# ShawnHuang497/MedPLIB

Hardware: AMD Instinct MI355X
Metric: train samples/sec (img+64tok) (higher is better)
Workload: dtype bf16

## Files before the change

### include/medplib_hip.h

```cpp
#ifndef MEDPLIB_HIP_H
#define MEDPLIB_HIP_H
#include <stddef.h>
#include <stdint.h>

#ifdef __cplusplus
extern "C" {
#endif

typedef struct ihipStream_t* hipStream_t;

#define MP_OK 0
#define MP_ERR_SHAPE (-1)
#define MP_ERR_DTYPE (-2)
#define MP_ERR_WORKSPACE (-3)
#define MP_ERR_LAUNCH (-4)
#define MP_ERR_ARG (-5)
#define MP_BF16 0
#define MP_F32 1
#define MP_ACT_NONE 0
#define MP_ACT_RELU 1
#define MP_ACT_GELU 2
#define MP_ACT_QUICK_GELU 3
#define MP_ACT_SILU 4
#define MP_ACT_SWIGLU_PAIR 5
// ... 48 lines not shown
#define MP_POS_ERR_CACHE 2
int mp_gemv_rmsnorm_rope_append_bounded_bf16(const void* x, int64_t ldx, const float* norm_w, float eps, const void* W_qkv, int64_t ldw,
                                             void* qkv, int64_t ldy, const float* cos_t, const float* sin_t, void* cache_k, void* cache_v,
                                             const int* pos_dev, int M, int heads, int head_dim, int K, int64_t cache_batch_stride,
                                             int64_t cache_seq_stride, int table_rows, int cache_rows, int* err, hipStream_t stream);

int mp_gemm_set_workspace(void* ws, int64_t ws_bytes, int* tickets, int n_tickets);
int mp_gemm_set_stream_workspace(hipStream_t stream, void* ws, int64_t ws_bytes, int* tickets, int n_tickets);

int mp_attention_fwd_bf16(const void* Q, int64_t q_sb, int64_t q_ss, const void* K, int64_t k_sb, int64_t k_ss,
                          const void* V, int64_t v_sb, int64_t v_ss, void* O, int64_t o_sb, int64_t o_ss,
                          const uint8_t* key_valid, const float* rel_h, const float* rel_w, int kh, int kw, int B, int H,
                          int Sq, int Sk, int D, int causal, float scale, int variant, const int* sk_dev, hipStream_t stream);

int mp_rmsnorm_bf16(const void* x, int64_t ldx, const float* w, void* y, int64_t ldy, int64_t rows, int dim, float eps,
                    hipStream_t stream);
int mp_layernorm_bf16(const void* x, int64_t ldx, const float* w, const float* b, void* y, int64_t ldy, int64_t rows,
                      int dim, float eps, hipStream_t stream);
int mp_rope_qk_bf16(void* qkv, int64_t ld, const float* cos_t, const float* sin_t, int64_t tokens, int seq, int heads,
                    int head_dim, int pos_offset, hipStream_t stream);
int mp_rope_qk_bounded_bf16(void* qkv, int64_t ld, const float* cos_t, const float* sin_t, int64_t tokens, int seq, int heads,
                            int head_dim, int pos_offset, int table_rows, hipStream_t stream);
int mp_decode_rope_append_bf16(void* qkv, int64_t ld, const float* cos_t, const float* sin_t, void* cache_k, void* cache_v,
                               const int* pos_dev, int B, int heads, int head_dim, int64_t cache_batch_stride, int64_t cache_seq_stride,
                               hipStream_t stream);
int mp_decode_rope_append_bounded_bf16(void* qkv, int64_t ld, const float* cos_t, const float* sin_t, void* cache_k, void* cache_v,
                                       const int* pos_dev, int B, int heads, int head_dim, int64_t cache_batch_stride,
                                       int64_t cache_seq_stride, int table_rows, int cache_rows, int* err, hipStream_t stream);
int mp_advance_ints(int* p, int n, int delta, hipStream_t stream);
int mp_argmax_rows_f32(const float* x, int64_t ld, int64_t rows, int cols, int64_t* out, hipStream_t stream);
int mp_sample_rows_f32(const float* logits, int64_t ld, int64_t rows, int cols, float inv_temperature, const float* u, int64_t* out,
// ... 109 lines not shown
int mp_decode_norm_gate_route(const void* x, int64_t ldx, const float* ln_w, float eps, const float* wg, void* h, int64_t ldh,
                              const float* rts_uniform, int tokens, int dim, int n_experts, int capacity, float* gates, int* expert,
                              int* slot, float* weight, int* kept_counts, long long* exp_counts, float* l_aux, hipStream_t stream);
int mp_decode_norm_gate_route_top2(const void* x, int64_t ldx, const float* ln_w, float eps, const float* wg, void* h, int64_t ldh,
                                   const float* noise, int tokens, int dim, int n_experts, int capacity, int* expert, int* slot,
                                   float* weight, int* kept_counts, long long* exp_counts, float* l_aux, hipStream_t stream);
int mp_moe_residual_mix_bf16(const void* x, const void* moe, const void* mlp, const void* coef, int64_t ldcoef, void* out,
                             int64_t tokens, int dim, hipStream_t stream);
int mp_moe_route_top2(const float* gates, const float* logits, const float* noise, int tokens, int n_experts, int capacity,
                      int* expert, int* slot, float* weight, int* kept_counts, long long* exp_counts, float* l_aux,
                      hipStream_t stream);
int mp_gate_noise_f32(float* out, int64_t n, uint64_t seed, uint64_t offset, int gumbel, hipStream_t stream);
int mp_gate_noise_dev_f32(float* out, int64_t n, uint64_t seed, const int* pass_dev, uint64_t stride, int gumbel, hipStream_t stream);
int mp_rmsnorm_gate_bf16(const void* x, int64_t ldx, const float* ln_w, float eps, void* h, int64_t ldh, const float* wg, float* logits,
                         float* gates, int64_t tokens, int dim, int n_experts, hipStream_t stream);
int mp_rmsnorm_gate_rstd_bf16(const void* x, int64_t ldx, const float* ln_w, float eps, const float* wg, float* logits, float* gates,
                              float* rstd, int64_t tokens, int dim, int n_experts, hipStream_t stream);
int mp_gemm_qkv_rope_scaled_bf16(const void* A, int64_t lda, const void* Wi, int64_t ldw, void* C, int64_t ldc, const float* cos_t,
                                 const float* sin_t, const float* row_scale, int M, int N, int K, int seq, int pos_offset, int head_dim,
                                 hipStream_t stream);
int mp_gemm_qkv_rope_scaled_bounded_bf16(const void* A, int64_t lda, const void* Wi, int64_t ldw, void* C, int64_t ldc, const float* cos_t,
                                         const float* sin_t, const float* row_scale, int M, int N, int K, int seq, int pos_offset,
                                         int head_dim, int table_rows, hipStream_t stream);
int mp_gemm_bf16_nt_batched_rows_scaled(const void* A, int64_t lda, const int* a_rows, const float* a_row_scale, const void* W, int64_t ldw,
                                        int64_t strideW, void* C, int64_t ldc, int64_t strideC, int rows_stride, int batch, int M, int N,
                                        int K, const int* m_dev, hipStream_t stream);
int mp_gemm_fold_ok(int M, int N, int K);
int mp_moe_dispatch_bf16(const void* x, int64_t ldx, const int* expert, const int* slot, void* buf, int64_t ldbuf, int64_t tokens, int dim,
                         int capacity, int top_k, hipStream_t stream);
int mp_moe_combine_bf16(const void* y, const int* expert, const int* slot, const float* weight, const void* residual, void* out,
// ... 114 lines not shown
```

### medplib_amd/csrc/ce_moe.hip

```cpp
#include "common.h"
#include <algorithm>

namespace {

constexpr int MAXE = 8;

__global__ __launch_bounds__(256) void ce_rows_kernel(const float* __restrict__ logits, int64_t ld, const int64_t* __restrict__ labels,
                                                      int V, float* __restrict__ row_loss) {
  __shared__ float red[16];
  const int64_t r = blockIdx.x;
  const float* x = logits + r * ld;
  float m = -INFINITY;
  for (int i = threadIdx.x; i < V; i += 256) m = fmaxf(m, x[i]);
  m = block_max(m, red);
  float s = 0.f;
  for (int i = threadIdx.x; i < V; i += 256) s += expf(x[i] - m);
  s = block_sum(s, red);
  if (threadIdx.x == 0) row_loss[r] = logf(s) + m - x[labels[r]];
}

__global__ __launch_bounds__(256) void mean_plus_kernel(const float* __restrict__ x, int64_t n, float scale, const float* __restrict__ add,
                                                        int n_add, float add_scale, float* __restrict__ out) {
  __shared__ float red[16];
  float s = 0.f;
// ... 39 lines not shown
        for (int j = 0; j < 8; ++j) acc[e] = fmaf((float)v[j], w[j], acc[e]);
      }
    }
  }
  moe_gate_finish(acc, E, lane, logits_out, gates_out);
}

__global__ __launch_bounds__(256) void moe_gate_kernel(const bf16_t* __restrict__ x, int64_t ldx, const float* __restrict__ wg,
                                                       float* __restrict__ logits, float* __restrict__ gates, int64_t T, int d, int E) {
  const int lane = threadIdx.x & 63;
  const int64_t tok = (int64_t)blockIdx.x * 4 + (threadIdx.x >> 6);
  if (tok >= T) return;
  moe_gate_token(x + tok * ldx, wg, d, E, lane, logits + tok * E, gates + tok * E);
}

template <int NCH, bool LDSW>
__global__ __launch_bounds__(512) void rmsnorm_gate_kernel(const bf16_t* __restrict__ x, int64_t ldx, const float* __restrict__ w, float eps,
                                                           bf16_t* __restrict__ h, int64_t ldh, const float* __restrict__ wg, int E,
                                                           float* __restrict__ logits, float* __restrict__ gates, int64_t T, float* __restrict__ rstd = nullptr) {
  extern __shared__ __attribute__((aligned(16))) float wsh[];
  constexpr int dim = NCH * 512;
  const int lane = threadIdx.x & 63;
  const int nwv = blockDim.x >> 6, step4 = blockDim.x * 4;
  if constexpr (LDSW) {
    for (int i = threadIdx.x * 4; i < dim; i += step4) *reinterpret_cast<f32x4*>(wsh + i) = *reinterpret_cast<const f32x4*>(w + i);
    for (int i = threadIdx.x * 4; i < E * dim; i += step4) *reinterpret_cast<f32x4*>(wsh + dim + i) = *reinterpret_cast<const f32x4*>(wg + i);
    __syncthreads();
  }
  const float* wn = LDSW ? wsh : w;
  const float* wgs = LDSW ? wsh + dim : wg;
  for (int64_t tok = (int64_t)blockIdx.x * nwv + (threadIdx.x >> 6); tok < T; tok += (int64_t)gridDim.x * nwv) {
    const bf16_t* xr = x + tok * ldx;
    bf16x8 v[NCH];
    float part[4] = {0.f, 0.f, 0.f, 0.f};
#pragma unroll
    for (int k = 0; k < NCH; ++k) {
      v[k] = *reinterpret_cast<const bf16x8*>(xr + (k * 64 + lane) * 8);
#pragma unroll
      for (int j = 0; j < 8; ++j) { const float f = (float)v[k][j]; part[k & 3] += f * f; }
    }
    float ss = 0.f;
#pragma unroll
    for (int wv = 0; wv < 4; ++wv) ss += wave_sum(part[wv]);
    const float rs = rsqrtf(ss / (float)dim + eps);
    if (rstd && lane == 0) rstd[tok] = rs;
    if (!h && E == 0) continue;
    float acc[MAXE];
#pragma unroll
    for (int e = 0; e < MAXE; ++e) acc[e] = 0.f;
    bf16_t* hr = h + tok * ldh;
#pragma unroll
    for (int k = 0; k < NCH; ++k) {
// ... 20 lines not shown
    float mx = -INFINITY;
#pragma unroll
    for (int e = 0; e < MAXE; ++e)
      if (e < E) { acc[e] = wave_sum(acc[e]); mx = fmaxf(mx, acc[e]); }
    if (lane == 0) {
      float sum = 0.f, pr[MAXE];
#pragma unroll
      for (int e = 0; e < MAXE; ++e)
        if (e < E) { pr[e] = expf(acc[e] - mx); sum += pr[e]; }
#pragma unroll
      for (int e = 0; e < MAXE; ++e)
        if (e < E) {
          if (logits) logits[tok * E + e] = acc[e];
          gates[tok * E + e] = pr[e] / sum;
        }
    }
  }
}

template <bool FAST>
__global__ __launch_bounds__(1024) void moe_route_top1_kernel(const float* __restrict__ gates, const float* __restrict__ rts, int T,
                                                              int E, int capacity, int* __restrict__ expert, int* __restrict__ slot,
                                                              float* __restrict__ weight, int* __restrict__ kept_counts,
                                                              long long* __restrict__ exp_counts, float* __restrict__ l_aux,
                                                              int* __restrict__ slot_token) {
  __shared__ float red[16];
  __shared__ int cnt_sh[MAXE];
  __shared__ int scan[16][MAXE];
  const int tid = threadIdx.x;
  if (tid < MAXE) cnt_sh[tid] = 0;
  __syncthreads();
  float me[MAXE];
  int cnt[MAXE];
#pragma unroll
  for (int e = 0; e < MAXE; ++e) { me[e] = 0.f; cnt[e] = 0; }
  const int chunk = (T + 1023) / 1024;
  const int s0 = min(T, tid * chunk), s1 = min(T, s0 + chunk);
  int ex[FAST ? 16 : 1];
  if constexpr (FAST) {
    float bvv[16];
// ... 40 lines not shown
    }
  }
  float aux = 0.f;
  for (int e = 0; e < E; ++e) {
    float m = 0.f; int c = 0;
#pragma unroll
    for (int k = 0; k < MAXE; ++k) if (k == e) { m = me[k]; c = cnt[k]; }
    const float msum = block_sum(m, red);
    int cw = c;
#pragma unroll
    for (int off = 1; off < 64; off <<= 1) cw += __shfl_xor(cw, off, 64);
    if ((tid & 63) == 0 && cw) atomicAdd(&cnt_sh[e], cw);
    __syncthreads();
    aux += (msum / (float)T) * ((float)cnt_sh[e] / (float)T);
  }
  if (tid == 0) {
    l_aux[0] = aux * (float)E;
    for (int e = 0; e < E; ++e) exp_counts[e] = cnt_sh[e];
  }
  __syncthreads();
  const int lane = tid & 63, wv = tid >> 6;
  bool over = false;
  for (int e = 0; e < E; ++e) over |= cnt_sh[e] > capacity;
  const bool via_memory = !FAST || (rts && over);
  if (via_memory) {
    for (int s = tid; s < T; s += 1024) slot[s] = 1;
    __syncthreads();
  }
  if (rts && over) {
    __shared__ unsigned hist[256];
    __shared__ unsigned bin_suf[256], bin_tot[4];
// ... 158 lines not shown
    }
    if (kp) {
      int v = 0;
#pragma unroll
      for (int k = 0; k < MAXE; ++k) if (k == e) { v = base[k]; base[k] += 1; }
      slot[s] = (v < capacity) ? v : -1;
      if (slot_token && v < capacity) slot_token[(int64_t)e * capacity + v] = s;
    } else {
      slot[s] = -1;
    }
  }
  if (tid == 1023)
    for (int e = 0; e < E; ++e) kept_counts[e] = min(base[e], capacity);
}

__device__ __forceinline__ void moe_route_top1_small_body(const float* __restrict__ gates, const float* __restrict__ rts, int T,
                                                               int E, int capacity, int* __restrict__ expert, int* __restrict__ slot,
                                                                  float* __restrict__ weight, int* __restrict__ kept_counts,
                                                                  long long* __restrict__ exp_counts, float* __restrict__ l_aux,
                                                                  int* __restrict__ slot_token, int s) {
  const bool live = s < T;
  int best = 0;
  float bv = live ? gates[(int64_t)s * E] : 0.f;
  float aux = 0.f;
  for (int e = 1; e < E; ++e) {
    const float g = live ? gates[(int64_t)s * E + e] : 0.f;
    if (g > bv) { bv = g; best = e; }
  }
  for (int e = 0; e < E; ++e) {
    const float me = wave_sum(live ? gates[(int64_t)s * E + e] : 0.f) / (float)T;
// ... 425 lines not shown
extern "C" int mp_mean_plus_f32(const float* x, int64_t n, float scale, const float* add, int n_add, float add_scale, float* out,
                                hipStream_t stream) {
  hipLaunchKernelGGL(mean_plus_kernel, dim3(1), dim3(256), 0, stream, x, n, scale, add, n_add, add_scale, out);
  return mp_check_launch("mp_mean_plus_f32");
}

extern "C" int mp_moe_gate_bf16(const void* x, int64_t ldx, const float* wg, float* logits, float* gates, int64_t tokens, int dim,
                                int n_experts, hipStream_t stream) {
  MP_REQUIRE(n_experts >= 1 && n_experts <= MAXE && dim % 8 == 0 && ldx % 8 == 0, MP_ERR_SHAPE, "mp_moe_gate_bf16: bad shape (E<=8)");
  if (tokens == 0) return MP_OK;
  hipLaunchKernelGGL(moe_gate_kernel, dim3((unsigned)mp_cdiv(tokens, 4)), dim3(256), 0, stream, (const bf16_t*)x, ldx, wg, logits,
                     gates, tokens, dim, n_experts);
  return mp_check_launch("mp_moe_gate_bf16");
}

static int rmsnorm_gate_launch(const void* x, int64_t ldx, const float* ln_w, float eps, void* h, int64_t ldh, const float* wg,
                                    float* logits, float* gates, int64_t tokens, int dim, int n_experts, float* rstd, hipStream_t stream) {
  MP_REQUIRE(n_experts >= 0 && n_experts <= MAXE && ldx % 8 == 0 && ldh % 8 == 0, MP_ERR_SHAPE, "mp_rmsnorm_gate_bf16: bad shape (E <= %d)", MAXE);
  MP_REQUIRE(dim == 2048 || dim == 4096 || dim == 8192, MP_ERR_SHAPE, "mp_rmsnorm_gate_bf16: dim %d (2048, 4096 or 8192)", dim);
  MP_REQUIRE(n_experts == 0 || (wg != nullptr && gates != nullptr), MP_ERR_ARG, "mp_rmsnorm_gate_bf16: gate outputs missing");
  if (tokens == 0) return MP_OK;
  const size_t lds = (size_t)(1 + n_experts) * dim * sizeof(float);
  const bool stage = lds <= 65536;
  static int rg_waves = -1;
  if (rg_waves < 0) { const char* e = getenv("MP_RG_WAVES"); rg_waves = (e && atoi(e) == 8) ? 8 : 4; }
  const int nwv = (stage && tokens >= 2048) ? rg_waves : 4;
  const dim3 grid((unsigned)std::min<int64_t>(mp_cdiv(tokens, nwv), stage ? (nwv == 8 ? 768 : 512) : (1 << 30))), blk(64 * nwv);
#define MP_RG(N)                                                                                                                                   \
  do {                                                                                                                                             \
    if (stage) hipLaunchKernelGGL((rmsnorm_gate_kernel<N, true>), grid, blk, lds, stream, (const bf16_t*)x, ldx, ln_w, eps, (bf16_t*)h, ldh, wg,   \
                                  n_experts, logits, gates, tokens, rstd);                                                                               \
    else hipLaunchKernelGGL((rmsnorm_gate_kernel<N, false>), grid, blk, 0, stream, (const bf16_t*)x, ldx, ln_w, eps, (bf16_t*)h, ldh, wg,          \
                            n_experts, logits, gates, tokens, rstd);                                                                                     \
  } while (0)
  if (dim == 2048) MP_RG(4); else if (dim == 4096) MP_RG(8); else MP_RG(16);
#undef MP_RG
  return mp_check_launch("mp_rmsnorm_gate_bf16");
}

extern "C" int mp_rmsnorm_gate_bf16(const void* x, int64_t ldx, const float* ln_w, float eps, void* h, int64_t ldh, const float* wg, float* logits,
                                    float* gates, int64_t tokens, int dim, int n_experts, hipStream_t stream) {
  MP_REQUIRE(h != nullptr, MP_ERR_ARG, "mp_rmsnorm_gate_bf16: h is null (mp_rmsnorm_gate_rstd_bf16 is the form without the normalised rows)");
  return rmsnorm_gate_launch(x, ldx, ln_w, eps, h, ldh, wg, logits, gates, tokens, dim, n_experts, nullptr, stream);
}

extern "C" int mp_rmsnorm_gate_rstd_bf16(const void* x, int64_t ldx, const float* ln_w, float eps, const float* wg, float* logits, float* gates,
                                         float* rstd, int64_t tokens, int dim, int n_experts, hipStream_t stream) {
  MP_REQUIRE(rstd != nullptr && ln_w != nullptr, MP_ERR_ARG, "mp_rmsnorm_gate_rstd_bf16: rstd and ln_w required");
  return rmsnorm_gate_launch(x, ldx, ln_w, eps, nullptr, 8, wg, logits, gates, tokens, dim, n_experts, rstd, stream);
}

extern "C" int mp_moe_route_top1(const float* gates, const float* rts_uniform, int tokens, int n_experts, int capacity, int* expert,
                                 int* slot, float* weight, int* kept_counts, long long* exp_counts, float* l_aux, int* slot_token,
                                 hipStream_t stream) {
  MP_REQUIRE(n_experts >= 1 && n_experts <= MAXE && tokens > 0 && capacity >= 0, MP_ERR_SHAPE, "mp_moe_route_top1: bad shape");
  if (tokens <= 64) {
    hipLaunchKernelGGL(moe_route_top1_small_kernel, dim3(1), dim3(64), 0, stream, gates, rts_uniform, tokens, n_experts, capacity, expert,
                       slot, weight, kept_counts, exp_counts, l_aux, slot_token);
    return mp_check_launch("mp_moe_route_top1(small)");
  }
  if (tokens <= 16 * 1024)
    hipLaunchKernelGGL(moe_route_top1_kernel<true>, dim3(1), dim3(1024), 0, stream, gates, rts_uniform, tokens, n_experts, capacity, expert,
                       slot, weight, kept_counts, exp_counts, l_aux, slot_token);
  else
    hipLaunchKernelGGL(moe_route_top1_kernel<false>, dim3(1), dim3(1024), 0, stream, gates, rts_uniform, tokens, n_experts, capacity, expert,
                       slot, weight, kept_counts, exp_counts, l_aux, slot_token);
  return mp_check_launch("mp_moe_route_top1");
}

extern "C" int mp_decode_norm_gate_route(const void* x, int64_t ldx, const float* ln_w, float eps, const float* wg, void* h, int64_t ldh,
                                        const float* rts_uniform, int tokens, int dim, int n_experts, int capacity, float* gates,
                                        int* expert, int* slot, float* weight, int* kept_counts, long long* exp_counts, float* l_aux,
                                        hipStream_t stream) {
  MP_REQUIRE(tokens >= 1 && tokens <= 8 && n_experts >= 1 && n_experts <= MAXE && dim % 8 == 0 && dim <= 8192 && ldx % 8 == 0 &&
                 ldh % 8 == 0 && capacity >= 0,
             MP_ERR_SHAPE, "mp_decode_norm_gate_route: tokens <= 8, experts <= %d, dim %% 8 == 0 and <= 8192", MAXE);
  hipLaunchKernelGGL(decode_norm_gate_route_kernel, dim3(1), dim3(256), 0, stream, (const bf16_t*)x, ldx, ln_w, eps, wg, (bf16_t*)h, ldh,
                     rts_uniform, tokens, dim, n_experts, capacity, gates, expert, slot, weight, kept_counts, exp_counts, l_aux);
  return mp_check_launch("mp_decode_norm_gate_route");
}

extern "C" int mp_decode_norm_gate_route_top2(const void* x, int64_t ldx, const float* ln_w, float eps, const float* wg, void* h, int64_t ldh,
// ... 78 lines not shown
```

### medplib_amd/csrc/norm_elementwise.hip

```cpp
#include "common.h"

namespace {

constexpr int ROW_THREADS = 256;
constexpr int MAXC = 4;

__global__ __launch_bounds__(ROW_THREADS) void rmsnorm_bf16_kernel(const bf16_t* __restrict__ x, const float* __restrict__ w,
                                                                   bf16_t* __restrict__ y, int dim, float eps,
                                                                   int64_t ldx, int64_t ldy) {
  __shared__ float red[16];
  const int64_t row = blockIdx.x;
  const bf16_t* xr = x + row * ldx;
  bf16_t* yr = y + row * ldy;
  bf16x8 v[MAXC];
  float ss = 0.f;
#pragma unroll
  for (int c = 0; c < MAXC; ++c) {
    const int i = (c * ROW_THREADS + threadIdx.x) * 8;
    if (i < dim) {
      v[c] = *reinterpret_cast<const bf16x8*>(xr + i);
#pragma unroll
      for (int j = 0; j < 8; ++j) { const float f = (float)v[c][j]; ss += f * f; }
    }
  }
  ss = block_sum(ss, red);
  const float rs = rsqrtf(ss / (float)dim + eps);
// ... 301 lines not shown
}

}

extern "C" int mp_argmax_rows_f32(const float* x, int64_t ld, int64_t rows, int cols, int64_t* out, hipStream_t stream) {
  MP_REQUIRE(cols > 0, MP_ERR_SHAPE, "mp_argmax_rows_f32: bad shape");
  if (rows == 0) return MP_OK;
  if (cols <= 32768)
    hipLaunchKernelGGL(argmax_rows_wide_kernel, dim3((unsigned)rows), dim3(1024), 0, stream, x, ld, cols, out);
  else
    hipLaunchKernelGGL(argmax_rows_kernel, dim3((unsigned)rows), dim3(256), 0, stream, x, ld, cols, out);
  return mp_check_launch("mp_argmax_rows_f32");
}

extern "C" int mp_rmsnorm_bf16(const void* x, int64_t ldx, const float* w, void* y, int64_t ldy, int64_t rows, int dim,
                               float eps, hipStream_t stream) {
  MP_REQUIRE(dim % 8 == 0 && dim <= ROW_THREADS * 8 * MAXC && ldx % 8 == 0 && ldy % 8 == 0, MP_ERR_SHAPE,
             "mp_rmsnorm_bf16: dim=%d unsupported", dim);
  if (rows == 0) return MP_OK;
  hipLaunchKernelGGL(rmsnorm_bf16_kernel, dim3((unsigned)rows), dim3(ROW_THREADS), 0, stream, (const bf16_t*)x, w,
                     (bf16_t*)y, dim, eps, ldx, ldy);
  return mp_check_launch("mp_rmsnorm_bf16");
}

extern "C" int mp_layernorm_bf16(const void* x, int64_t ldx, const float* w, const float* b, void* y, int64_t ldy,
                                 int64_t rows, int dim, float eps, hipStream_t stream) {
  MP_REQUIRE(dim % 8 == 0 && dim <= ROW_THREADS * 8 * MAXC && ldx % 8 == 0 && ldy % 8 == 0, MP_ERR_SHAPE,
             "mp_layernorm_bf16: dim=%d unsupported", dim);
  if (rows == 0) return MP_OK;
  if (dim <= 2048) {
    hipLaunchKernelGGL(layernorm_bf16_wave_kernel, dim3((unsigned)mp_cdiv(rows, 4)), dim3(256), 0, stream, (const bf16_t*)x, w, b,
                       (bf16_t*)y, rows, dim, eps, ldx, ldy);
    return mp_check_launch("mp_layernorm_bf16");
  }
  hipLaunchKernelGGL(layernorm_bf16_kernel, dim3((unsigned)rows), dim3(ROW_THREADS), 0, stream, (const bf16_t*)x, w, b,
                     (bf16_t*)y, dim, eps, ldx, ldy);
// ... 101 lines not shown
```

### medplib_amd/model/llama.py

```python
import math

import torch

from .. import ops


def _rope_tables(seq, head_dim, theta, device, start=0):
    inv = 1.0 / (theta ** (torch.arange(0, head_dim, 2, dtype=torch.float32) / head_dim))
    freqs = torch.outer(torch.arange(start, seq, dtype=torch.float32), inv)
    return freqs.cos().contiguous().to(device), freqs.sin().contiguous().to(device)


ROPE_GROW_ROWS = 1024


def rope_rows_for(n, rows):
    return rows if n <= rows else -(-n // ROPE_GROW_ROWS) * ROPE_GROW_ROWS


class LlamaStack:
    def __init__(self, cfg, device, init_std=0.02, seed=0):
        self.cfg, self.device = cfg, device
        d, ff, L, V = cfg.hidden_size, cfg.intermediate_size, cfg.num_hidden_layers, cfg.vocab_size
        E = cfg.num_experts
# ... 134 lines not shown
        if self.rts_uniform_provider is not None:
            return self.rts_uniform_provider(i, T, E)
        if not self.cfg.moe_gate_sampling:
            return None
        L = len(self.layers)
        pass_dev = self._pass_dev
        key = (self.gate_pass, T, E, bool(gumbel), pass_dev is not None)
        if getattr(self, "_draws_key", None) != key:
            if pass_dev is not None:
                self._draws_all = ops.gate_noise_dev(L * T * E, self.cfg.moe_gate_seed, pass_dev, L * T * E, gumbel, self.device)
            else:
                self._draws_all = ops.gate_noise(L * T * E, self.cfg.moe_gate_seed, self.gate_pass * L * T * E, gumbel, self.device)
            self._draws_key = key
        return self._draws_all[i * T * E:(i + 1) * T * E]

    def _mlp(self, i, lw, h, x, gate=None, needed=None, rstd=None):
        cfg = self.cfg
        T = x.shape[0]
        if i not in self.moe_layers:
            if T <= 8:
                return ops.gemv(ops.gemv(h, lw["gu"], act=ops.ACT_SWIGLU_PAIR), lw["down"], residual=x), None, None
            act = ops.gemm(h, lw["gu"], act=ops.ACT_SWIGLU_PAIR)
            return ops.gemm(act, lw["down"], residual=x), None, None
        E, ff, d = cfg.num_experts, cfg.intermediate_size, cfg.hidden_size
        cap = self.capacity(T)
        k = cfg.top_k_experts
        logits, gates = gate if gate is not None else ops.moe_gate(h, lw["wg"])
        if k == 1 and self.ep is None and T <= 8 and not cfg.use_residual:
            draws = None if cap >= T else self._gate_draws(i, T, E, gumbel=False)
            expert, slot, weight, kept, counts, l_aux = ops.moe_route_top1(gates, cap, draws)
            act = ops.gemv(h, lw["gu"], act=ops.ACT_SWIGLU_PAIR, w_index=expert)
            out = ops.gemv(act, lw["down"], residual=x, w_index=expert, row_scale=weight, row_keep=slot)
            return out, l_aux, (expert, slot, counts)
        if k == 2 and self.ep is None and T <= 8 and not cfg.use_residual:
            expert, slot, weight, kept, counts, l_aux = ops.moe_route_top2(gates, logits, cap, self._gate_draws(i, T, E, gumbel=True))
            act = ops.gemv_top2_gate_up(h, lw["gu"], expert, slot)
            return ops.gemv_top2_down(act, lw["down"], expert, slot, weight, x), l_aux, (expert, slot, counts)
        if k == 1 and self.ep is None and self.fuse_moe_gather_scatter and not cfg.use_residual:
            expert, slot, weight, kept, counts, l_aux, slot_token = ops.moe_route_top1(
                gates, cap, self._gate_draws(i, T, E, gumbel=False), want_slot_token=True)
            act = torch.empty((E, cap, ff), dtype=torch.bfloat16, device=x.device)
            if needed is not None:
                self.pruned_rows = int(getattr(self, "needed_rows")[0].numel())
                slot_token, kept = ops.moe_filter_slots(slot_token, kept, needed)
            if ops.GEMM_TIMER is not None:
                ops.GEMM_TIMER.batched_tag = i
            ev = getattr(self, "layer_events", None)
            if ev is not None and i < len(ev):
                ev[i].record()
            if rstd is not None:
                ops.gemm_batched_rows(x, lw["gu_f"], act, kept, a_rows=slot_token, act=ops.ACT_SWIGLU_PAIR, rows_stride=cap, a_row_scale=rstd)
            else:
                ops.gemm_batched_rows(h, lw["gu"], act, kept, a_rows=slot_token, act=ops.ACT_SWIGLU_PAIR, rows_stride=cap)
            ops.gemm_batched_rows(act, lw["down"], x, kept, c_rows=slot_token, c_scale=weight, residual=x, rows_stride=cap)
# ... 98 lines not shown
            else:
                qkv = lin(h, lw["qkv"])
                ops.rope_qk_(qkv, self.cos, self.sin, S, H, D, pos_offset=pos0)
            q5 = qkv.unflatten(0, (B, S)).unflatten(2, (3, H, D))
            if kv_cache is not None:
                kv_cache["k"][i][:, pos0:pos0 + S].copy_(q5[:, :, 1])
                kv_cache["v"][i][:, pos0:pos0 + S].copy_(q5[:, :, 2])
            if kv_cache is not None and pos0 > 0:
                assert S == 1 and key_valid is None, "cached decode is single-token, un-padded (the reference evaluates with batch 1)"
                attn = ops.attention(q5[:, :, 0], kv_cache["k"][i][:, :pos0 + 1], kv_cache["v"][i][:, :pos0 + 1], causal=False)
            else:
                attn = ops.attention(q5[:, :, 0], q5[:, :, 1], q5[:, :, 2], causal=True, key_valid=key_valid)
            x = lin(attn.view(B * S, d), lw["o"], residual=x)
            x_gate_in = x.clone() if (collect_routing and i in self.moe_layers) else None
            if i in self.moe_layers and d in ops.RMSNORM_GATE_DIMS and B * S > 8:
                h, lg, gt = ops.rmsnorm_gate(x, lw["ln2"], cfg.rms_norm_eps, lw["wg"])
                x, l_aux, r = self._mlp(i, lw, h, x, gate=(lg, gt), needed=needed_mask if i == len(self.layers) - 1 else None)
            else:
                h = ops.rmsnorm(x, lw["ln2"], cfg.rms_norm_eps)
                x, l_aux, r = self._mlp(i, lw, h, x, needed=needed_mask if (i in self.moe_layers and i == len(self.layers) - 1) else None)
            if l_aux is not None:
                aux.append(l_aux)
                if collect_routing:
                    routing.append(r)
                    gate_inputs.append(x_gate_in)
        if kv_cache is not None:
            kv_cache["len"] = pos0 + S
        out = ops.rmsnorm(x, self.norm_w, cfg.rms_norm_eps)
        if collect_routing:
            self.last_gate_inputs = gate_inputs
        return out.view(B, S, d), aux, (routing if collect_routing else None)

    def decode_step(self, emb, kv_cache, counters, pass_dev=None):
        self._pass_dev = pass_dev
        try:
            return self._decode_step(emb, kv_cache, counters)
        finally:
            self._pass_dev = None

    def _decode_step(self, emb, kv_cache, counters):
        cfg = self.cfg
        B, _, d = emb.shape
        H, D = cfg.num_attention_heads, cfg.head_dim
# ... 53 lines not shown
```

### medplib_amd/ops.py

```python
import torch

from ._lib import lib

BF16, F32 = 0, 1
ACT_NONE, ACT_RELU, ACT_GELU, ACT_QUICK_GELU, ACT_SILU, ACT_SWIGLU_PAIR = 0, 1, 2, 3, 4, 5
SACT_NONE, SACT_RELU, SACT_GELU, SACT_SIGMOID = 0, 1, 2, 3


def _stream():
    return torch.cuda.current_stream().cuda_stream


def _p(t):
    return None if t is None else t.data_ptr()


def _chk(t, dtype, name):
    if not t.is_cuda:
        raise ValueError(f"{name}: expected a GPU tensor (medplib_amd has no CPU path)")
    if t.dtype != dtype:
        raise TypeError(f"{name}: expected {dtype}, got {t.dtype}")


def _dt(dtype):
# ... 622 lines not shown
    return cos_t.shape[0], cache_k.shape[1], err


def decode_rope_append(qkv, cos_t, sin_t, cache_k, cache_v, pos_dev, heads, head_dim, err=None):
    _chk(qkv, torch.bfloat16, "decode_rope_append.qkv"); _chk(pos_dev, torch.int32, "decode_rope_append.pos")
    assert qkv.dim() == 2 and qkv.stride(1) == 1 and cache_k.stride(3) == 1 and cache_k.stride(2) == head_dim
    table_rows, cache_rows, err = _decode_bounds(cos_t, sin_t, cache_k, cache_v, err)
    lib().call("mp_decode_rope_append_bounded_bf16", _p(qkv), qkv.stride(0), _p(cos_t), _p(sin_t), _p(cache_k), _p(cache_v), _p(pos_dev),
               qkv.shape[0], heads, head_dim, cache_k.stride(0), cache_k.stride(1), table_rows, cache_rows, _p(err), _stream())


def advance_ints(t, delta=1):
    lib().call("mp_advance_ints", _p(t), t.numel(), int(delta), _stream())


def rmsnorm(x, w, eps, out=None):
    _chk(x, torch.bfloat16, "rmsnorm.x"); _chk(w, torch.float32, "rmsnorm.w")
    x2 = x.reshape(-1, x.shape[-1]); assert x2.stride(1) == 1
    if out is None:
        out = torch.empty_like(x2)
    lib().call("mp_rmsnorm_bf16", _p(x2), x2.stride(0), _p(w), _p(out), out.stride(0), x2.shape[0], x2.shape[1], float(eps),
               _stream())
    return out.view(x.shape)


def layernorm(x, w, b, eps, out=None):
    _chk(x, torch.bfloat16, "layernorm.x"); _chk(w, torch.float32, "layernorm.w")
    x2 = x.reshape(-1, x.shape[-1]); assert x2.stride(1) == 1
    if out is None:
        out = torch.empty_like(x2)
    lib().call("mp_layernorm_bf16", _p(x2), x2.stride(0), _p(w), _p(b), _p(out), out.stride(0), x2.shape[0], x2.shape[1],
               float(eps), _stream())
    return out.view(x.shape)


def rope_qk_(qkv, cos_t, sin_t, seq, heads, head_dim, pos_offset=0):
    _chk(qkv, torch.bfloat16, "rope.qkv"); _chk(cos_t, torch.float32, "rope.cos"); _chk(sin_t, torch.float32, "rope.sin")
# ... 635 lines not shown
def moe_route_top1(gates, capacity, rts_uniform=None, want_slot_token=False):
    T, E = gates.shape
    dev = gates.device
    slot_token = torch.empty((E, int(capacity)), dtype=torch.int32, device=dev) if want_slot_token else None
    expert = torch.empty(T, dtype=torch.int32, device=dev); slot = torch.empty(T, dtype=torch.int32, device=dev)
    weight = torch.empty(T, dtype=torch.float32, device=dev)
    kept = torch.empty(E, dtype=torch.int32, device=dev); counts = torch.empty(E, dtype=torch.int64, device=dev)
    l_aux = torch.empty(1, dtype=torch.float32, device=dev)
    lib().call("mp_moe_route_top1", _p(gates), _p(rts_uniform), T, E, int(capacity), _p(expert), _p(slot), _p(weight), _p(kept),
               _p(counts), _p(l_aux), _p(slot_token), _stream())
    if want_slot_token:
        return expert, slot, weight, kept, counts, l_aux, slot_token
    return expert, slot, weight, kept, counts, l_aux


def decode_norm_gate_route(x, ln_w, eps, wg, capacity, rts_uniform=None):
    _chk(x, torch.bfloat16, "decode_norm_gate_route.x"); _chk(ln_w, torch.float32, "decode_norm_gate_route.ln_w")
    _chk(wg, torch.float32, "decode_norm_gate_route.wg")
    T, d = x.shape
    E = wg.shape[0]
    dev = x.device
    h = torch.empty((T, d), dtype=torch.bfloat16, device=dev)
    expert = torch.empty(T, dtype=torch.int32, device=dev); slot = torch.empty(T, dtype=torch.int32, device=dev)
    weight = torch.empty(T, dtype=torch.float32, device=dev)
    kept = torch.empty(E, dtype=torch.int32, device=dev); counts = torch.empty(E, dtype=torch.int64, device=dev)
    l_aux = torch.empty(1, dtype=torch.float32, device=dev)
    lib().call("mp_decode_norm_gate_route", _p(x), x.stride(0), _p(ln_w), float(eps), _p(wg), _p(h), h.stride(0), _p(rts_uniform), T, d, E,
               int(capacity), None, _p(expert), _p(slot), _p(weight), _p(kept), _p(counts), _p(l_aux), _stream())
    return h, expert, slot, weight, kept, counts, l_aux

# ... 202 lines not shown
```

Measured before the change: 138.0.

## Fuse top-1 MoE routing into rmsnorm-gate kernel and normalize only needed rows

Extends the rmsnorm+gate kernel with a ROUTE variant that computes argmax expert, weight and per-workgroup count/gate-sum partials in the same pass. A new multi-block ranges kernel then derives global counts, aux loss and capacity slots with ballot-based ranking, falling back to the serial router when random token selection is needed. Each workgroup now owns a contiguous row range and prefetches its first row before staging weights. The final rmsnorm takes an optional row index list so only the needed rows are normalized. This removes a separate single-block routing pass and some final-norm work, at the cost of a workspace buffer and more complex partitioning logic.

New measurement: 137.9 (median of 2 runs). Within noise of the previous version (-0.0%).

```diff
diff --git a/include/medplib_hip.h b/include/medplib_hip.h
--- a/include/medplib_hip.h
+++ b/include/medplib_hip.h
@@ -86,7 +86,7 @@
                           int Sq, int Sk, int D, int causal, float scale, int variant, const int* sk_dev, hipStream_t stream);
 
 int mp_rmsnorm_bf16(const void* x, int64_t ldx, const float* w, void* y, int64_t ldy, int64_t rows, int dim, float eps,
-                    hipStream_t stream);
+                    const int64_t* row_idx, hipStream_t stream);
 int mp_layernorm_bf16(const void* x, int64_t ldx, const float* w, const float* b, void* y, int64_t ldy, int64_t rows,
                       int dim, float eps, hipStream_t stream);
 int mp_rope_qk_bf16(void* qkv, int64_t ld, const float* cos_t, const float* sin_t, int64_t tokens, int seq, int heads,
@@ -226,6 +226,12 @@
 int mp_gate_noise_dev_f32(float* out, int64_t n, uint64_t seed, const int* pass_dev, uint64_t stride, int gumbel, hipStream_t stream);
 int mp_rmsnorm_gate_bf16(const void* x, int64_t ldx, const float* ln_w, float eps, void* h, int64_t ldh, const float* wg, float* logits,
                          float* gates, int64_t tokens, int dim, int n_experts, hipStream_t stream);
+#define MP_ROUTE_MAX_WGS 1024
+#define MP_ROUTE_WS_BYTES (MP_ROUTE_MAX_WGS * 8 * 12)
+int mp_rmsnorm_gate_route_top1_bf16(const void* x, int64_t ldx, const float* ln_w, float eps, void* h, int64_t ldh, const float* wg,
+                                    float* logits, float* gates, const float* rts_uniform, int tokens, int dim, int n_experts,
+                                    int capacity, int* expert, int* slot, float* weight, int* kept_counts, long long* exp_counts,
+                                    float* l_aux, int* slot_token, void* workspace, int64_t workspace_bytes, hipStream_t stream);
 int mp_rmsnorm_gate_rstd_bf16(const void* x, int64_t ldx, const float* ln_w, float eps, const float* wg, float* logits, float* gates,
                               float* rstd, int64_t tokens, int dim, int n_experts, hipStream_t stream);
 int mp_gemm_qkv_rope_scaled_bf16(const void* A, int64_t lda, const void* Wi, int64_t ldw, void* C, int64_t ldc, const float* cos_t,
diff --git a/medplib_amd/csrc/ce_moe.hip b/medplib_amd/csrc/ce_moe.hip
--- a/medplib_amd/csrc/ce_moe.hip
+++ b/medplib_amd/csrc/ce_moe.hip
@@ -4,6 +4,8 @@
 namespace {
 
 constexpr int MAXE = 8;
+constexpr int MP_ROUTE_MAX_WGS = 1024;
+constexpr int64_t MP_ROUTE_WS_BYTES = (int64_t)MP_ROUTE_MAX_WGS * MAXE * 12;
 
 __global__ __launch_bounds__(256) void ce_rows_kernel(const float* __restrict__ logits, int64_t ld, const int64_t* __restrict__ labels,
                                                       int V, float* __restrict__ row_loss) {
@@ -77,14 +79,31 @@
   moe_gate_token(x + tok * ldx, wg, d, E, lane, logits + tok * E, gates + tok * E);
 }
 
-template <int NCH, bool LDSW>
+struct RoutePartials {
+  int* expert;
+  float* weight;
+  int* cnt;
+  double* gsum;
+};
+
+template <int NCH, bool LDSW, bool ROUTE>
 __global__ __launch_bounds__(512) void rmsnorm_gate_kernel(const bf16_t* __restrict__ x, int64_t ldx, const float* __restrict__ w, float eps,
                                                            bf16_t* __restrict__ h, int64_t ldh, const float* __restrict__ wg, int E,
-                                                           float* __restrict__ logits, float* __restrict__ gates, int64_t T, float* __restrict__ rstd = nullptr) {
+                                                           float* __restrict__ logits, float* __restrict__ gates, int64_t T, int rows_wg,
+                                                           float* __restrict__ rstd, RoutePartials rp) {
   extern __shared__ __attribute__((aligned(16))) float wsh[];
+  __shared__ int cnt_wv[8][MAXE];
+  __shared__ double gsum_wv[8][MAXE];
   constexpr int dim = NCH * 512;
   const int lane = threadIdx.x & 63;
   const int nwv = blockDim.x >> 6, step4 = blockDim.x * 4;
+  const int64_t row_end = min(T, ((int64_t)blockIdx.x + 1) * rows_wg);
+  int64_t tok = (int64_t)blockIdx.x * rows_wg + (threadIdx.x >> 6);
+  bf16x8 v[NCH];
+  if (tok < row_end) {
+#pragma unroll
+    for (int k = 0; k < NCH; ++k) v[k] = *reinterpret_cast<const bf16x8*>(x + tok * ldx + (k * 64 + lane) * 8);
+  }
   if constexpr (LDSW) {
     for (int i = threadIdx.x * 4; i < dim; i += step4) *reinterpret_cast<f32x4*>(wsh + i) = *reinterpret_cast<const f32x4*>(w + i);
     for (int i = threadIdx.x * 4; i < E * dim; i += step4) *reinterpret_cast<f32x4*>(wsh + dim + i) = *reinterpret_cast<const f32x4*>(wg + i);
@@ -92,13 +111,16 @@
   }
   const float* wn = LDSW ? wsh : w;
   const float* wgs = LDSW ? wsh + dim : wg;
-  for (int64_t tok = (int64_t)blockIdx.x * nwv + (threadIdx.x >> 6); tok < T; tok += (int64_t)gridDim.x * nwv) {
+  int rcnt[MAXE];
+  double rsum[MAXE];
+#pragma unroll
+  for (int e = 0; e < MAXE; ++e) { rcnt[e] = 0; rsum[e] = 0.0; }
+  for (bool first = true; tok < row_end; tok += nwv, first = false) {
     const bf16_t* xr = x + tok * ldx;
-    bf16x8 v[NCH];
     float part[4] = {0.f, 0.f, 0.f, 0.f};
 #pragma unroll
     for (int k = 0; k < NCH; ++k) {
-      v[k] = *reinterpret_cast<const bf16x8*>(xr + (k * 64 + lane) * 8);
+      if (!first) v[k] = *reinterpret_cast<const bf16x8*>(xr + (k * 64 + lane) * 8);
 #pragma unroll
       for (int j = 0; j < 8; ++j) { const float f = (float)v[k][j]; part[k & 3] += f * f; }
     }
@@ -149,16 +171,46 @@
           if (logits) logits[tok * E + e] = acc[e];
           gates[tok * E + e] = pr[e] / sum;
         }
+      if constexpr (ROUTE) {
+        int best = 0;
+        float bv = pr[0] / sum;
+#pragma unroll
+        for (int e = 0; e < MAXE; ++e)
+          if (e < E) {
+            const float g = pr[e] / sum;
+            if (e > 0 && g > bv) { bv = g; best = e; }
+            rsum[e] += (double)g;
+          }
+        rp.expert[tok] = best;
+        rp.weight[tok] = bv;
+#pragma unroll
+        for (int e = 0; e < MAXE; ++e) rcnt[e] += (e == best);
+      }
+    }
+  }
+  if constexpr (ROUTE) {
+    const int wv = threadIdx.x >> 6;
+    if (lane == 0) {
+#pragma unroll
+      for (int e = 0; e < MAXE; ++e) { cnt_wv[wv][e] = rcnt[e]; gsum_wv[wv][e] = rsum[e]; }
+    }
+    __syncthreads();
+    if ((int)threadIdx.x < E) {
+      int c = 0;
+      double g = 0.0;
+      for (int k = 0; k < nwv; ++k) { c += cnt_wv[k][threadIdx.x]; g += gsum_wv[k][threadIdx.x]; }
+      rp.cnt[(int64_t)blockIdx.x * E + threadIdx.x] = c;
+      rp.gsum[(int64_t)blockIdx.x * E + threadIdx.x] = g;
     }
   }
 }
 
 template <bool FAST>
-__global__ __launch_bounds__(1024) void moe_route_top1_kernel(const float* __restrict__ gates, const float* __restrict__ rts, int T,
-                                                              int E, int capacity, int* __restrict__ expert, int* __restrict__ slot,
-                                                              float* __restrict__ weight, int* __restrict__ kept_counts,
-                                                              long long* __restrict__ exp_counts, float* __restrict__ l_aux,
-                                                              int* __restrict__ slot_token) {
+__device__ __forceinline__ void moe_route_top1_body(const float* __restrict__ gates, const float* __restrict__ rts, int T,
+                                                    int E, int capacity, int* __restrict__ expert, int* __restrict__ slot,
+                                                    float* __restrict__ weight, int* __restrict__ kept_counts,
+                                                    long long* __restrict__ exp_counts, float* __restrict__ l_aux,
+                                                    int* __restrict__ slot_token) {
   __shared__ float red[16];
   __shared__ int cnt_sh[MAXE];
   __shared__ int scan[16][MAXE];
@@ -229,7 +281,7 @@
     __syncthreads();
     aux += (msum / (float)T) * ((float)cnt_sh[e] / (float)T);
   }
-  if (tid == 0) {
+  if (tid == 0 && l_aux) {
     l_aux[0] = aux * (float)E;
     for (int e = 0; e < E; ++e) exp_counts[e] = cnt_sh[e];
   }
@@ -418,6 +470,93 @@
     for (int e = 0; e < E; ++e) kept_counts[e] = min(base[e], capacity);
 }
 
+template <bool FAST>
+__global__ __launch_bounds__(1024) void moe_route_top1_kernel(const float* __restrict__ gates, const float* __restrict__ rts, int T,
+                                                              int E, int capacity, int* __restrict__ expert, int* __restrict__ slot,
+                                                              float* __restrict__ weight, int* __restrict__ kept_counts,
+                                                              long long* __restrict__ exp_counts, float* __restrict__ l_aux,
+                                                              int* __restrict__ slot_token) {
+  moe_route_top1_body<FAST>(gates, rts, T, E, capacity, expert, slot, weight, kept_counts, exp_counts, l_aux, slot_token);
+}
+
+__global__ __launch_bounds__(1024) void moe_route_ranges_kernel(const float* __restrict__ gates, const float* __restrict__ rts, int T, int E,
+                                                                int capacity, const int* __restrict__ pcnt, const double* __restrict__ pgsum,
+                                                                int n_part, int rows_wg, int wgs_per, int* __restrict__ expert,
+                                                                int* __restrict__ slot, float* __restrict__ weight,
+                                                                int* __restrict__ kept_counts, long long* __restrict__ exp_counts,
+                                                                float* __restrict__ l_aux, int* __restrict__ slot_token) {
+  __shared__ int tot_sh[MAXE], base_sh[MAXE];
+  __shared__ int wtot[16][MAXE];
+  __shared__ double dred[16];
+  const int tid = threadIdx.x, lane = tid & 63, wv = tid >> 6;
+  const int part0 = blockIdx.x * wgs_per;
+  if (tid < MAXE) { tot_sh[tid] = 0; base_sh[tid] = 0; }
+  __syncthreads();
+  for (int e = 0; e < E; ++e) {
+    int tot = 0, base = 0;
+    for (int g = tid; g < n_part; g += 1024) {
+      const int c = pcnt[(int64_t)g * E + e];
+      tot += c;
+      if (g < part0) base += c;
+    }
+#pragma unroll
+    for (int off = 1; off < 64; off <<= 1) { tot += __shfl_xor(tot, off, 64); base += __shfl_xor(base, off, 64); }
+    if (lane == 0) {
+      if (tot) atomicAdd(&tot_sh[e], tot);
+      if (base) atomicAdd(&base_sh[e], base);
+    }
+  }
+  __syncthreads();
+  bool over = false;
+  for (int e = 0; e < E; ++e) over |= tot_sh[e] > capacity;
+  const bool select = rts != nullptr && over;
+  if (blockIdx.x == 0) {
+    float aux = 0.f;
+    for (int e = 0; e < E; ++e) {
+      double m = 0.0;
+      for (int g = tid; g < n_part; g += 1024) m += pgsum[(int64_t)g * E + e];
+#pragma unroll
+      for (int off = 1; off < 64; off <<= 1) m += __shfl_xor(m, off, 64);
+      if (lane == 0) dred[wv] = m;
+      __syncthreads();
+      double ms = 0.0;
+      for (int k = 0; k < 16; ++k) ms += dred[k];
+      __syncthreads();
+      aux += ((float)ms / (float)T) * ((float)tot_sh[e] / (float)T);
+    }
+    if (tid == 0) {
+      l_aux[0] = aux * (float)E;
+      for (int e = 0; e < E; ++e) {
+        exp_counts[e] = tot_sh[e];
+        if (!select) kept_counts[e] = min(tot_sh[e], capacity);
+      }
+    }
+  }
+  if (select) {
+    if (blockIdx.x != 0) return;
+    if (T <= 16 * 1024) moe_route_top1_body<true>(gates, rts, T, E, capacity, expert, slot, weight, kept_counts, nullptr, nullptr, slot_token);
+    else moe_route_top1_body<false>(gates, rts, T, E, capacity, expert, slot, weight, kept_counts, nullptr, nullptr, slot_token);
+    return;
+  }
+  const int64_t s0 = (int64_t)part0 * rows_wg;
+  const int64_t s = s0 + tid;
+  const bool live = tid < wgs_per * rows_wg && s < T;
+  const int ex = live ? expert[s] : -1;
+  int rank = 0;
+  for (int e = 0; e < E; ++e) {
+    const unsigned long long m = __ballot(ex == e);
+    if (ex == e) rank = __popcll(m & ((1ull << lane) - 1ull));
+    if (lane == 0) wtot[wv][e] = __popcll(m);
+  }
+  __syncthreads();
+  if (live) {
+    rank += base_sh[ex];
+    for (int k = 0; k < wv; ++k) rank += wtot[k][ex];
+    slot[s] = rank < capacity ? rank : -1;
+    if (slot_token && rank < capacity) slot_token[(int64_t)ex * capacity + rank] = (int)s;
+  }
+}
+
 __device__ __forceinline__ void moe_route_top1_small_body(const float* __restrict__ gates, const float* __restrict__ rts, int T,
                                                                int E, int capacity, int* __restrict__ expert, int* __restrict__ slot,
                                                                   float* __restrict__ weight, int* __restrict__ kept_counts,
@@ -873,40 +1012,56 @@
   return mp_check_launch("mp_moe_gate_bf16");
 }
 
+struct RgShape { bool stage; int nwv, rows_wg; unsigned grid; size_t lds; };
+static RgShape rmsnorm_gate_shape(int64_t tokens, int dim, int n_experts, int64_t max_wgs) {
+  RgShape sh;
+  sh.lds = (size_t)(1 + n_experts) * dim * sizeof(float);
+  sh.stage = sh.lds <= 65536;
+  static int rg_waves = -1;
+  if (rg_waves < 0) { const char* e = getenv("MP_RG_WAVES"); rg_waves = (e && atoi(e) == 8) ? 8 : 4; }
+  sh.nwv = (sh.stage && tokens >= 2048) ? rg_waves : 4;
+  const int64_t wgs = std::min<int64_t>(mp_cdiv(tokens, sh.nwv), sh.stage ? (sh.nwv == 8 ? 768 : 512) : max_wgs);
+  sh.rows_wg = (int)mp_cdiv(tokens, wgs);
+  sh.grid = (unsigned)mp_cdiv(tokens, sh.rows_wg);
+  if (!sh.stage) sh.lds = 0;
+  return sh;
+}
+
 static int rmsnorm_gate_launch(const void* x, int64_t ldx, const float* ln_w, float eps, void* h, int64_t ldh, const float* wg,
-                                    float* logits, float* gates, int64_t tokens, int dim, int n_experts, float* rstd, hipStream_t stream) {
+                                    float* logits, float* gates, int64_t tokens, int dim, int n_experts, float* rstd, const RgShape& sh,
+                                    const RoutePartials* rp, hipStream_t stream) {
   MP_REQUIRE(n_experts >= 0 && n_experts <= MAXE && ldx % 8 == 0 && ldh % 8 == 0, MP_ERR_SHAPE, "mp_rmsnorm_gate_bf16: bad shape (E <= %d)", MAXE);
   MP_REQUIRE(dim == 2048 || dim == 4096 || dim == 8192, MP_ERR_SHAPE, "mp_rmsnorm_gate_bf16: dim %d (2048, 4096 or 8192)", dim);
   MP_REQUIRE(n_experts == 0 || (wg != nullptr && gates != nullptr), MP_ERR_ARG, "mp_rmsnorm_gate_bf16: gate outputs missing");
   if (tokens == 0) return MP_OK;
-  const size_t lds = (size_t)(1 + n_experts) * dim * sizeof(float);
-  const bool stage = lds <= 65536;
-  static int rg_waves = -1;
-  if (rg_waves < 0) { const char* e = getenv("MP_RG_WAVES"); rg_waves = (e && atoi(e) == 8) ? 8 : 4; }
-  const int nwv = (stage && tokens >= 2048) ? rg_waves : 4;
-  const dim3 grid((unsigned)std::min<int64_t>(mp_cdiv(tokens, nwv), stage ? (nwv == 8 ? 768 : 512) : (1 << 30))), blk(64 * nwv);
+  const dim3 grid(sh.grid), blk(64 * sh.nwv);
+  const RoutePartials none = {nullptr, nullptr, nullptr, nullptr};
+#define MP_RG_K(N, S, R)                                                                                                                           \
+  hipLaunchKernelGGL((rmsnorm_gate_kernel<N, S, R>), grid, blk, sh.lds, stream, (const bf16_t*)x, ldx, ln_w, eps, (bf16_t*)h, ldh, wg, n_experts,   \
+                     logits, gates, tokens, sh.rows_wg, rstd, rp ? *rp : none)
 #define MP_RG(N)                                                                                                                                   \
   do {                                                                                                                                             \
-    if (stage) hipLaunchKernelGGL((rmsnorm_gate_kernel<N, true>), grid, blk, lds, stream, (const bf16_t*)x, ldx, ln_w, eps, (bf16_t*)h, ldh, wg,   \
-                                  n_experts, logits, gates, tokens, rstd);                                                                               \
-    else hipLaunchKernelGGL((rmsnorm_gate_kernel<N, false>), grid, blk, 0, stream, (const bf16_t*)x, ldx, ln_w, eps, (bf16_t*)h, ldh, wg,          \
-                            n_experts, logits, gates, tokens, rstd);                                                                                     \
+    if (rp) { if (sh.stage) MP_RG_K(N, true, true); else MP_RG_K(N, false, true); }                                                                \
+    else { if (sh.stage) MP_RG_K(N, true, false); else MP_RG_K(N, false, false); }                                                                 \
   } while (0)
   if (dim == 2048) MP_RG(4); else if (dim == 4096) MP_RG(8); else MP_RG(16);
 #undef MP_RG
+#undef MP_RG_K
   return mp_check_launch("mp_rmsnorm_gate_bf16");
 }
 
 extern "C" int mp_rmsnorm_gate_bf16(const void* x, int64_t ldx, const float* ln_w, float eps, void* h, int64_t ldh, const float* wg, float* logits,
                                     float* gates, int64_t tokens, int dim, int n_experts, hipStream_t stream) {
   MP_REQUIRE(h != nullptr, MP_ERR_ARG, "mp_rmsnorm_gate_bf16: h is null (mp_rmsnorm_gate_rstd_bf16 is the form without the normalised rows)");
-  return rmsnorm_gate_launch(x, ldx, ln_w, eps, h, ldh, wg, logits, gates, tokens, dim, n_experts, nullptr, stream);
+  return rmsnorm_gate_launch(x, ldx, ln_w, eps, h, ldh, wg, logits, gates, tokens, dim, n_experts, nullptr,
+                             rmsnorm_gate_shape(tokens, dim, n_experts, (int64_t)1 << 30), nullptr, stream);
 }
 
 extern "C" int mp_rmsnorm_gate_rstd_bf16(const void* x, int64_t ldx, const float* ln_w, float eps, const float* wg, float* logits, float* gates,
                                          float* rstd, int64_t tokens, int dim, int n_experts, hipStream_t stream) {
   MP_REQUIRE(rstd != nullptr && ln_w != nullptr, MP_ERR_ARG, "mp_rmsnorm_gate_rstd_bf16: rstd and ln_w required");
-  return rmsnorm_gate_launch(x, ldx, ln_w, eps, nullptr, 8, wg, logits, gates, tokens, dim, n_experts, rstd, stream);
+  return rmsnorm_gate_launch(x, ldx, ln_w, eps, nullptr, 8, wg, logits, gates, tokens, dim, n_experts, rstd,
+                             rmsnorm_gate_shape(tokens, dim, n_experts, (int64_t)1 << 30), nullptr, stream);
 }
 
 extern "C" int mp_moe_route_top1(const float* gates, const float* rts_uniform, int tokens, int n_experts, int capacity, int* expert,
@@ -925,6 +1080,28 @@
     hipLaunchKernelGGL(moe_route_top1_kernel<false>, dim3(1), dim3(1024), 0, stream, gates, rts_uniform, tokens, n_experts, capacity, expert,
                        slot, weight, kept_counts, exp_counts, l_aux, slot_token);
   return mp_check_launch("mp_moe_route_top1");
+}
+
+extern "C" int mp_rmsnorm_gate_route_top1_bf16(const void* x, int64_t ldx, const float* ln_w, float eps, void* h, int64_t ldh, const float* wg,
+                                               float* logits, float* gates, const float* rts_uniform, int tokens, int dim, int n_experts,
+                                               int capacity, int* expert, int* slot, float* weight, int* kept_counts, long long* exp_counts,
+                                               float* l_aux, int* slot_token, void* workspace, int64_t workspace_bytes, hipStream_t stream) {
+  MP_REQUIRE(h != nullptr && n_experts >= 1 && n_experts <= MAXE && tokens > 0 && capacity >= 0, MP_ERR_SHAPE, "mp_rmsnorm_gate_route_top1_bf16: bad shape");
+  MP_REQUIRE(workspace != nullptr && workspace_bytes >= MP_ROUTE_WS_BYTES && (uintptr_t)workspace % 8 == 0, MP_ERR_WORKSPACE,
+             "mp_rmsnorm_gate_route_top1_bf16: workspace of MP_ROUTE_WS_BYTES, 8-byte aligned");
+  const RgShape sh = rmsnorm_gate_shape(tokens, dim, n_experts, MP_ROUTE_MAX_WGS);
+  MP_REQUIRE(sh.rows_wg <= 1024 && sh.grid <= MP_ROUTE_MAX_WGS, MP_ERR_SHAPE, "mp_rmsnorm_gate_route_top1_bf16: too many tokens (%d)", tokens);
+  RoutePartials rp;
+  rp.expert = expert; rp.weight = weight;
+  rp.gsum = (double*)workspace;
+  rp.cnt = (int*)((char*)workspace + (size_t)MP_ROUTE_MAX_WGS * MAXE * sizeof(double));
+  const int rc = rmsnorm_gate_launch(x, ldx, ln_w, eps, h, ldh, wg, logits, gates, tokens, dim, n_experts, nullptr, sh, &rp, stream);
+  if (rc != MP_OK) return rc;
+  const int wgs_per = 1024 / sh.rows_wg;
+  hipLaunchKernelGGL(moe_route_ranges_kernel, dim3((unsigned)mp_cdiv(sh.grid, wgs_per)), dim3(1024), 0, stream, gates, rts_uniform, tokens,
+                     n_experts, capacity, rp.cnt, rp.gsum, (int)sh.grid, sh.rows_wg, wgs_per, expert, slot, weight, kept_counts, exp_counts,
+                     l_aux, slot_token);
+  return mp_check_launch("mp_rmsnorm_gate_route_top1_bf16");
 }
 
 extern "C" int mp_decode_norm_gate_route(const void* x, int64_t ldx, const float* ln_w, float eps, const float* wg, void* h, int64_t ldh,
diff --git a/medplib_amd/csrc/norm_elementwise.hip b/medplib_amd/csrc/norm_elementwise.hip
--- a/medplib_amd/csrc/norm_elementwise.hip
+++ b/medplib_amd/csrc/norm_elementwise.hip
@@ -7,9 +7,9 @@
 
 __global__ __launch_bounds__(ROW_THREADS) void rmsnorm_bf16_kernel(const bf16_t* __restrict__ x, const float* __restrict__ w,
                                                                    bf16_t* __restrict__ y, int dim, float eps,
-                                                                   int64_t ldx, int64_t ldy) {
+                                                                   int64_t ldx, int64_t ldy, const int64_t* __restrict__ row_idx) {
   __shared__ float red[16];
-  const int64_t row = blockIdx.x;
+  const int64_t row = row_idx ? row_idx[blockIdx.x] : (int64_t)blockIdx.x;
   const bf16_t* xr = x + row * ldx;
   bf16_t* yr = y + row * ldy;
   bf16x8 v[MAXC];
@@ -341,12 +341,12 @@
 }
 
 extern "C" int mp_rmsnorm_bf16(const void* x, int64_t ldx, const float* w, void* y, int64_t ldy, int64_t rows, int dim,
-                               float eps, hipStream_t stream) {
+                               float eps, const int64_t* row_idx, hipStream_t stream) {
   MP_REQUIRE(dim % 8 == 0 && dim <= ROW_THREADS * 8 * MAXC && ldx % 8 == 0 && ldy % 8 == 0, MP_ERR_SHAPE,
              "mp_rmsnorm_bf16: dim=%d unsupported", dim);
   if (rows == 0) return MP_OK;
   hipLaunchKernelGGL(rmsnorm_bf16_kernel, dim3((unsigned)rows), dim3(ROW_THREADS), 0, stream, (const bf16_t*)x, w,
-                     (bf16_t*)y, dim, eps, ldx, ldy);
+                     (bf16_t*)y, dim, eps, ldx, ldy, row_idx);
   return mp_check_launch("mp_rmsnorm_bf16");
 }
 
diff --git a/medplib_amd/model/llama.py b/medplib_amd/model/llama.py
--- a/medplib_amd/model/llama.py
+++ b/medplib_amd/model/llama.py
@@ -172,7 +172,7 @@
             self._draws_key = key
         return self._draws_all[i * T * E:(i + 1) * T * E]
 
-    def _mlp(self, i, lw, h, x, gate=None, needed=None, rstd=None):
+    def _mlp(self, i, lw, h, x, gate=None, needed=None, rstd=None, routed=None):
         cfg = self.cfg
         T = x.shape[0]
         if i not in self.moe_layers:
@@ -195,7 +195,7 @@
             act = ops.gemv_top2_gate_up(h, lw["gu"], expert, slot)
             return ops.gemv_top2_down(act, lw["down"], expert, slot, weight, x), l_aux, (expert, slot, counts)
         if k == 1 and self.ep is None and self.fuse_moe_gather_scatter and not cfg.use_residual:
-            expert, slot, weight, kept, counts, l_aux, slot_token = ops.moe_route_top1(
+            expert, slot, weight, kept, counts, l_aux, slot_token = routed if routed is not None else ops.moe_route_top1(
                 gates, cap, self._gate_draws(i, T, E, gumbel=False), want_slot_token=True)
             act = torch.empty((E, cap, ff), dtype=torch.bfloat16, device=x.device)
             if needed is not None:
@@ -324,8 +324,13 @@
             x = lin(attn.view(B * S, d), lw["o"], residual=x)
             x_gate_in = x.clone() if (collect_routing and i in self.moe_layers) else None
             if i in self.moe_layers and d in ops.RMSNORM_GATE_DIMS and B * S > 8:
-                h, lg, gt = ops.rmsnorm_gate(x, lw["ln2"], cfg.rms_norm_eps, lw["wg"])
-                x, l_aux, r = self._mlp(i, lw, h, x, gate=(lg, gt), needed=needed_mask if i == len(self.layers) - 1 else None)
+                routed = None
+                if cfg.top_k_experts == 1 and self.ep is None and self.fuse_moe_gather_scatter and not cfg.use_residual:
+                    h, lg, gt, *routed = ops.rmsnorm_gate_route_top1(x, lw["ln2"], cfg.rms_norm_eps, lw["wg"], self.capacity(B * S),
+                                                                     self._gate_draws(i, B * S, cfg.num_experts, gumbel=False))
+                else:
+                    h, lg, gt = ops.rmsnorm_gate(x, lw["ln2"], cfg.rms_norm_eps, lw["wg"])
+                x, l_aux, r = self._mlp(i, lw, h, x, gate=(lg, gt), needed=needed_mask if i == len(self.layers) - 1 else None, routed=routed)
             else:
                 h = ops.rmsnorm(x, lw["ln2"], cfg.rms_norm_eps)
                 x, l_aux, r = self._mlp(i, lw, h, x, needed=needed_mask if (i in self.moe_layers and i == len(self.layers) - 1) else None)
@@ -336,7 +341,7 @@
                     gate_inputs.append(x_gate_in)
         if kv_cache is not None:
             kv_cache["len"] = pos0 + S
-        out = ops.rmsnorm(x, self.norm_w, cfg.rms_norm_eps)
+        out = ops.rmsnorm(x, self.norm_w, cfg.rms_norm_eps, rows=nr[0] if needed_mask is not None else None)
         if collect_routing:
             self.last_gate_inputs = gate_inputs
         return out.view(B, S, d), aux, (routing if collect_routing else None)
diff --git a/medplib_amd/ops.py b/medplib_amd/ops.py
--- a/medplib_amd/ops.py
+++ b/medplib_amd/ops.py
@@ -660,13 +660,16 @@
     lib().call("mp_advance_ints", _p(t), t.numel(), int(delta), _stream())
 
 
-def rmsnorm(x, w, eps, out=None):
+def rmsnorm(x, w, eps, out=None, rows=None):
     _chk(x, torch.bfloat16, "rmsnorm.x"); _chk(w, torch.float32, "rmsnorm.w")
     x2 = x.reshape(-1, x.shape[-1]); assert x2.stride(1) == 1
     if out is None:
         out = torch.empty_like(x2)
-    lib().call("mp_rmsnorm_bf16", _p(x2), x2.stride(0), _p(w), _p(out), out.stride(0), x2.shape[0], x2.shape[1], float(eps),
-               _stream())
+    n = x2.shape[0]
+    if rows is not None:
+        _chk(rows, torch.int64, "rmsnorm.rows"); assert rows.is_contiguous()
+        n = rows.numel()
+    lib().call("mp_rmsnorm_bf16", _p(x2), x2.stride(0), _p(w), _p(out), out.stride(0), n, x2.shape[1], float(eps), _p(rows), _stream())
     return out.view(x.shape)
 
 
@@ -1332,6 +1335,32 @@
     return expert, slot, weight, kept, counts, l_aux
 
 
+ROUTE_WS_BYTES = 1024 * 8 * 12
+
+
+def rmsnorm_gate_route_top1(x, ln_w, eps, wg, capacity, rts_uniform=None):
+    _chk(x, torch.bfloat16, "rmsnorm_gate_route_top1.x"); _chk(ln_w, torch.float32, "rmsnorm_gate_route_top1.w")
+    _chk(wg, torch.float32, "rmsnorm_gate_route_top1.wg")
+    T, d = x.shape
+    E = wg.shape[0]
+    assert x.stride(1) == 1 and wg.is_contiguous() and wg.shape[1] == d
+    if rts_uniform is not None:
+        _chk(rts_uniform, torch.float32, "rmsnorm_gate_route_top1.rts_uniform"); assert rts_uniform.is_contiguous() and rts_uniform.numel() == T * E
+    dev = x.device
+    h = torch.empty((T, d), dtype=torch.bfloat16, device=dev)
+    logits = torch.empty((T, E), dtype=torch.float32, device=dev); gates = torch.empty((T, E), dtype=torch.float32, device=dev)
+    slot_token = torch.empty((E, int(capacity)), dtype=torch.int32, device=dev)
+    expert = torch.empty(T, dtype=torch.int32, device=dev); slot = torch.empty(T, dtype=torch.int32, device=dev)
+    weight = torch.empty(T, dtype=torch.float32, device=dev)
+    kept = torch.empty(E, dtype=torch.int32, device=dev); counts = torch.empty(E, dtype=torch.int64, device=dev)
+    l_aux = torch.empty(1, dtype=torch.float32, device=dev)
+    ws = torch.empty(ROUTE_WS_BYTES // 8, dtype=torch.float64, device=dev)
+    lib().call("mp_rmsnorm_gate_route_top1_bf16", _p(x), x.stride(0), _p(ln_w), float(eps), _p(h), h.stride(0), _p(wg), _p(logits), _p(gates),
+               _p(rts_uniform), T, d, E, int(capacity), _p(expert), _p(slot), _p(weight), _p(kept), _p(counts), _p(l_aux), _p(slot_token),
+               _p(ws), ROUTE_WS_BYTES, _stream())
+    return h, logits, gates, expert, slot, weight, kept, counts, l_aux, slot_token
+
+
 def decode_norm_gate_route(x, ln_w, eps, wg, capacity, rts_uniform=None):
     _chk(x, torch.bfloat16, "decode_norm_gate_route.x"); _chk(ln_w, torch.float32, "decode_norm_gate_route.ln_w")
     _chk(wg, torch.float32, "decode_norm_gate_route.wg")
```
